# vitskvara/VBMatrixFactorization.jl

Hardware: AMD Instinct MI355X
Metric: VB iterations/sec (higher is better)
Workload: dtype bf16

## Files before the change

### vbmatrixfactorization.jl_amd/csrc/ctrl_kernels.hpp

```cpp
#pragma once
#include "common.hpp"
#include "blk_inverse.hpp"

namespace vbmf {

struct StateLayout {
    int Hp;
    __host__ __device__ long long n2() const { return (long long)Hp * Hp; }
    __host__ __device__ long long GA() const { return 0; }
    __host__ __device__ long long GB() const { return n2(); }
    __host__ __device__ long long GD() const { return 2 * n2(); }
    __host__ __device__ long long GX() const { return 3 * n2(); }
    __host__ __device__ long long SA() const { return 3 * n2() + 8; }
    __host__ __device__ long long SB() const { return 4 * n2() + 8; }
    __host__ __device__ long long KB() const { return 5 * n2() + 8; }
    __host__ __device__ long long W0() const { return 6 * n2() + 8; }
    __host__ __device__ long long W1() const { return 7 * n2() + 8; }
    __host__ __device__ long long W2() const { return 8 * n2() + 8; }
    __host__ __device__ long long ca() const { return 9 * n2() + 8; }
    __host__ __device__ long long cb() const { return 9 * n2() + 8 + Hp; }
    __host__ __device__ long long scal() const { return 9 * n2() + 8 + 2 * Hp; }
    __host__ __device__ long long total() const { return scal() + 32; }
};
enum : int { S_SIGMA2 = 0, S_TRYY, S_LOGDET_SA, S_LOGDET_SB, S_LAMB_PREV, S_LAMB_NEW, S_LAMD, S_D, S_ELBO,
// ... 429 lines not shown
        double theta = 0.0, theta_prev = 0.0, a0 = 0.0;
        bool again = false;
        for (int j = 0; j < kmax; ++j) {
            const float4* v4 = reinterpret_cast<const float4*>(&vbuf[cq * 16]);
            f32x2v a2[RB];
#pragma unroll
            for (int r = 0; r < RB; ++r) a2[r] = f32x2v{0.f, 0.f};
#pragma unroll
            for (int jj = 0; jj < 4; ++jj) {
                const float4 v = v4[jj];
                const f32x2v va = {v.x, v.y}, vb = {v.z, v.w};
#pragma unroll
                for (int r = 0; r < RB; ++r) {
                    a2[r] = __builtin_elementwise_fma(g[r][2 * jj], va, a2[r]);
                    a2[r] = __builtin_elementwise_fma(g[r][2 * jj + 1], vb, a2[r]);
                }
            }
            float acc[RB];
#pragma unroll
            for (int r = 0; r < RB; ++r) acc[r] = rowN_sum<NCQ>(a2[r][0] + a2[r][1]);
            float mine = acc[0];
            if constexpr (RB == 4) mine = (cq & 3) == 0 ? acc[0] : ((cq & 3) == 1 ? acc[1] : ((cq & 3) == 2 ? acc[2] : acc[3]));
            double wv = owner ? (double)mine : 0.0;
            const double alpha = block_sum_dpp<NT>(q * wv, red);
            wv = owner ? wv - alpha * q - beta * qp : 0.0;
            const double b2 = block_sum_dpp<NT>(wv * wv, red);
            const int k = j + 1;
            if (t == 0) { al[j] = alpha; be2[k] = b2; }
            if (j == 0) a0 = alpha;
            const bool brk = !(b2 > 1e-28) || !(b2 > EIG_LANCZOS_EXHAUSTED * a0 * a0);
            again = brk && k < kmax;
            qp = q;
            beta = sqrt(b2);
            q = brk ? 0.0 : wv / beta;
            if (owner) vbuf[myrow] = (float)q;
            __syncthreads();
            if (brk || k == next_look || k == kmax) {
                theta = tri_lambda_max(al, be2, k, theta_prev > 1e-9 ? theta_prev - 1e-9 : 0.0, 1.0 + 1e-6, imin, 4);
                if (brk || k == kmax || theta - theta_prev <= EIG_LANCZOS_TOL * theta) break;
                theta_prev = theta;
                next_look = k < 48 ? k + 12 : (k < 64 ? 64 : (k < 128 ? k + 32 : k + 64));
            }
        }
        best = theta > best ? theta : best;
        if (!again) break;
    }
    __syncthreads();
    return best;
}

constexpr int EIG_NSQ = 10;

template <int R>
__device__ __forceinline__ void eig_squaring_dev(double* __restrict__ st, StateLayout lay, int H, int spectral, int which,
                                        const int* __restrict__ ints, float* ldsf, int slot, bool check_stop = true) {
    __shared__ double red[16];
    __shared__ int s_arg;
    if (check_stop && load_stop(ints)) return;
    const int Hp = lay.Hp;
    const double* G = st + (which == 0 ? lay.GD() : lay.GB());
    double* scal = st + lay.scal();
    double tr = 0.0;
    for (int i = threadIdx.x; i < H; i += ctrl_nthreads()) tr += G[(long long)i * Hp + i];
    tr = block_sum(tr, red);
    if (!spectral || !(tr > 0.0) || !isfinite(tr)) {
        if (threadIdx.x == 0) scal[slot] = tr;
        return;
    }
    constexpr int T = 16, NP = T * R, LD = NP + 4;
    float* A0 = ldsf;
    float* A1 = ldsf + NP * LD;
    const int tx = threadIdx.x % T, ty = threadIdx.x / T;
    for (int t = threadIdx.x; t < NP * NP; t += ctrl_nthreads()) {
        const int i = t / NP, j = t - i * NP;
        A0[i * LD + j] = (i < H && j < H) ? (float)(G[(long long)i * Hp + j] / tr) : 0.f;
    }
    __syncthreads();
    float* cur = A0;
    float* nxt = A1;
    for (int sq = 0; sq < EIG_NSQ; ++sq) {
        float c[R][R];
#pragma unroll
        for (int a = 0; a < R; ++a)
#pragma unroll
            for (int b = 0; b < R; ++b) c[a][b] = 0.f;
        for (int k = 0; k < NP; k += 4) {
            float4 ai[R], bj[R];
#pragma unroll
            for (int a = 0; a < R; ++a) ai[a] = *reinterpret_cast<const float4*>(cur + (ty + T * a) * LD + k);
#pragma unroll
            for (int b = 0; b < R; ++b) bj[b] = *reinterpret_cast<const float4*>(cur + (tx + T * b) * LD + k);
#pragma unroll
            for (int a = 0; a < R; ++a)
#pragma unroll
                for (int b = 0; b < R; ++b) {
                    c[a][b] = fmaf(ai[a].x, bj[b].x, c[a][b]);
                    c[a][b] = fmaf(ai[a].y, bj[b].y, c[a][b]);
                    c[a][b] = fmaf(ai[a].z, bj[b].z, c[a][b]);
                    c[a][b] = fmaf(ai[a].w, bj[b].w, c[a][b]);
                }
        }
        double ss = 0.0;
#pragma unroll
        for (int a = 0; a < R; ++a)
#pragma unroll
            for (int b = 0; b < R; ++b) ss += (double)c[a][b] * (double)c[a][b];
        ss = block_sum(ss, red);
        const float sc = (ss > 0.0) ? (float)(1.0 / sqrt(ss)) : 0.f;
#pragma unroll
        for (int a = 0; a < R; ++a)
#pragma unroll
            for (int b = 0; b < R; ++b) nxt[(ty + T * a) * LD + tx + T * b] = c[a][b] * sc;
        __syncthreads();
        float* tmp = cur; cur = nxt; nxt = tmp;
        if (sq > 0 && fabs(ss - 1.0) < 1e-5) break;
    }
    if (threadIdx.x < 64) {
        float best = -1.f; int arg = 0;
        for (int i = threadIdx.x; i < H; i += 64) { const float v = cur[i * LD + i]; if (v > best) { best = v; arg = i; } }
        for (int off = 32; off > 0; off >>= 1) {
            const float ob = __shfl_down(best, off); const int oa = __shfl_down(arg, off);
            if (ob > best) { best = ob; arg = oa; }
        }
        if (threadIdx.x == 0) s_arg = arg;
    }
    __syncthreads();
    double num = 0.0, den = 0.0;
    {
        const int i = threadIdx.x >> 2, q = threadIdx.x & 3;
        for (int i0 = 0; i0 < H; i0 += 64) {
            const int row = i0 + i;
            if (row < H) {
                const int jn = (H + 3) / 4, j0 = q * jn, j1 = min(H, j0 + jn);
                double acc = 0.0;
                for (int j = j0; j < j1; ++j) acc += G[(long long)row * Hp + j] * (double)cur[j * LD + s_arg];
                const double vi = (double)cur[row * LD + s_arg];
                num += vi * acc;
                if (q == 0) den += vi * vi;
            }
        }
    }
    num = block_sum(num, red);
    den = block_sum(den, red);
    if (threadIdx.x == 0) scal[slot] = den > 0.0 ? num / den : 0.0;
    __syncthreads();
}

template <int R>
__device__ __forceinline__ void eig_dev(double* __restrict__ st, StateLayout lay, int H, int spectral, int which,
                                        const int* __restrict__ ints, float* ldsf, int slot, bool check_stop = true) {
    if (R <= 4 && __builtin_expect(!(spectral & 2), 1)) {
        eig_squaring_dev<R>(st, lay, H, spectral & 1, which, ints, ldsf, slot, check_stop);
    } else {
        __shared__ double red[16];
        if (check_stop && load_stop(ints)) return;
        const int Hp = lay.Hp;
        const double* G = st + (which == 0 ? lay.GD() : lay.GB());
        double* scal = st + lay.scal();
        double tr = 0.0;
        for (int i = threadIdx.x; i < H; i += ctrl_nthreads()) tr += G[(long long)i * Hp + i];
        tr = block_sum(tr, red);
        if (!(spectral & 1) || !(tr > 0.0) || !isfinite(tr)) {
            if (threadIdx.x == 0) scal[slot] = tr;
            return;
        }
        const double theta = lanczos_lambda_max<16 * R, 256>(G, Hp, H, tr, ldsf);
        if (threadIdx.x == 0) scal[slot] = tr * theta;
    }
}

template <int R>
__global__ __launch_bounds__(256) void eig_kernel(double* __restrict__ st, StateLayout lay, int H, int spectral,
                                                  int do_d, int do_b, const int* __restrict__ ints) {
    extern __shared__ __attribute__((aligned(16))) float lds_eig[];
    const int which = blockIdx.x;
    if ((which == 0 && !do_d) || (which == 1 && !do_b)) return;
    eig_dev<R>(st, lay, H, spectral, which, ints, lds_eig, which == 0 ? S_LAMD : S_LAMB_NEW);
}

__global__ __launch_bounds__(1024) void eig_lanczos_kernel(double* __restrict__ st, StateLayout lay, int H, int spectral,
                                                           int do_d, int do_b, const int* __restrict__ ints) {
    __shared__ double red[16];
    __shared__ __attribute__((aligned(16))) unsigned char lds_lz[EIG_LDS_BYTES];
    if (load_stop(ints)) return;
    const int which = blockIdx.x;
    if ((which == 0 && !do_d) || (which == 1 && !do_b)) return;
    const int Hp = lay.Hp;
    const double* G = st + (which == 0 ? lay.GD() : lay.GB());
    double* scal = st + lay.scal();
    const int slot = which == 0 ? S_LAMD : S_LAMB_NEW;
    double tr = 0.0;
    for (int i = threadIdx.x; i < H; i += (int)blockDim.x) tr += G[(long long)i * Hp + i];
    tr = block_sum(tr, red);
    if (!(spectral & 1) || !(tr > 0.0) || !isfinite(tr)) {
        if (threadIdx.x == 0) scal[slot] = tr;
        return;
    }
    const double theta = lanczos_lambda_max<256, 1024>(G, Hp, H, tr, lds_lz);
    if (threadIdx.x == 0) scal[slot] = tr * theta;
}

struct EndHandOff {
    double* img; int np;
    double sigma2, ca_h;
    bool live;
};
__device__ __forceinline__ void ctrl_end_dev(double* __restrict__ st, StateLayout lay, int H, double Lg, double M,
                                             int flags, double eps, double* __restrict__ trace,
                                             int* __restrict__ ints, int it_row, EndHandOff& ho, bool handoff,
                                             int* __restrict__ hw = nullptr) {
    __shared__ double red[16];
    __shared__ double sc_s[32];
    __shared__ double dg[4][256];
    const int Hp = lay.Hp;
    const double* GA = st + lay.GA();
    const double* GB = st + lay.GB();
    const double* SA = st + lay.SA();
    const double* SB = st + lay.SB();
    double* ca = st + lay.ca();
    double* cb = st + lay.cb();
    double* scal = st + lay.scal();
    int stopped = load_stop(ints);
    if ((flags & 64) && stopped == it_row + 1) stopped = 0;
    const int hme = threadIdx.x;
    const double scv = hme < 32 ? scal[hme] : 0.0;
    const double trdot = st[lay.GX()];
    double ca_h = hme < H ? ca[hme] : 1.0, cb_h = hme < H ? cb[hme] : 1.0;

    double t2 = 0.0;
    {
// ... 41 lines not shown
    ho.sigma2 = sigma2; ho.ca_h = ca_h;
    if (threadIdx.x == 0) {
        const double PI2 = 6.283185307179586476925286766559;
        double F = -(Lg * M / 2.0) * log(PI2 * sigma2) - resid / (2.0 * sigma2) + e;
        F += (M / 2.0) * sc_s[S_LOGDET_SA] + M * H / 2.0 + (Lg / 2.0) * sc_s[S_LOGDET_SB] + Lg * H / 2.0;
        scal[S_SIGMA2] = sigma2;
        scal[S_ELBO] = F;
        scal[S_RESID] = resid;
        scal[S_TRYBA] = trYBA;
        if (flags & 64) {
            if (trace) { trace[4 * it_row + 1] = sigma2; trace[4 * it_row + 2] = F; trace[4 * it_row + 3] = resid; }
        } else if (flags & 8) {
            const double d = sqrt(sc_s[S_LAMD] / sc_s[S_LAMB_PREV]);
            scal[S_D] = d;
            if (!(flags & 32)) scal[S_LAMB_PREV] = sc_s[S_LAMB_NEW];
            const int it = ints[I_ITERS];
            if (trace) { trace[4 * it + 0] = d; trace[4 * it + 1] = sigma2; trace[4 * it + 2] = F; trace[4 * it + 3] = resid; }
            ints[I_ITERS] = it + 1;
            const bool rerr = stop_on_remote_error(st, lay, ints);
            const bool stop = !(d > eps) || it + 1 >= ints[I_NITER] || rerr;
            if (stop) __hip_atomic_store(ints + I_STOP, 1, __ATOMIC_RELAXED, __HIP_MEMORY_SCOPE_AGENT);
            publish_loop_words(hw, ints, stop ? 1 : 0, it + 1);
        }
    }
    __syncthreads();
}

__device__ __forceinline__ void ctrl_end_dev(double* __restrict__ st, StateLayout lay, int H, double Lg, double M,
                                             int flags, double eps, double* __restrict__ trace,
                                             int* __restrict__ ints, int* __restrict__ hw) {
    EndHandOff none{nullptr, 0, 0.0, 1.0, false};
    ctrl_end_dev(st, lay, H, Lg, M, flags, eps, trace, ints, -1, none, false, hw);
}

__global__ __launch_bounds__(1024) void ctrl_end_kernel(double* __restrict__ st, StateLayout lay, int H, double Lg,
                                                       double M, int flags, double eps,
                                                       double* __restrict__ trace, int* __restrict__ ints,
                                                       int* __restrict__ hw) {
    ctrl_end_dev(st, lay, H, Lg, M, flags, eps, trace, ints, hw);
}

#ifndef VBMF_SEAM_STAMPS
#define VBMF_SEAM_STAMPS 0
#endif
template <int R>
__device__ __forceinline__ void cov_a_after_end_dev(double* __restrict__ st, StateLayout lay, int H, const EndHandOff& ho,
                                                    float* __restrict__ S32, int* __restrict__ ints) {
    constexpr int LD = 16 * R + 2;
#if VBMF_SEAM_STAMPS
    const unsigned long long s0 = wall_clock64();
#endif
    if ((int)threadIdx.x < H) ho.img[threadIdx.x * LD + threadIdx.x] += ho.sigma2 / ho.ca_h;
    double ldK; int badK;
#if VBMF_SEAM_STAMPS
    __syncthreads();
    const unsigned long long s1 = wall_clock64();
#endif
    spd_sweep_lds4<R>(ho.img, H, &ldK, &badK);
#if VBMF_SEAM_STAMPS
    __syncthreads();
    const unsigned long long s2 = wall_clock64();
#endif
    cov_store_lds4<R>(st, lay, H, 0, ho.sigma2, S32, ints, ho.img, ldK, badK, true);
#if VBMF_SEAM_STAMPS
    __syncthreads();
    if (threadIdx.x == 0) {
        unsigned long long* stamp = reinterpret_cast<unsigned long long*>(ints + 8);
        stamp[4] = s1 - s0; stamp[5] = s2 - s1; stamp[6] = wall_clock64() - s2;
    }
#endif
}

template <int R>
__device__ __forceinline__ void commit_cov_b_dev(double* __restrict__ st, StateLayout lay, int H, double M,
                                                 float* __restrict__ S32, int* __restrict__ ints, double* W) {
    if (load_stop(ints)) return;
#if VBMF_SEAM_STAMPS
    const unsigned long long s0 = wall_clock64();
#endif
    constexpr int NP = 16 * R, LD = NP + 2, U = 16;
    const int Hp = lay.Hp, sh = 31 - __clz(Hp), n = Hp * Hp;
    const double* src = st + lay.W0();
    const double* GA = st + lay.GA();
    const double* cb = st + lay.cb();
    double* dst = st + lay.SA();
    double* scal = st + lay.scal();
    const double sigma2 = scal[S_SIGMA2];
    const double cb_t = (int)threadIdx.x < H ? cb[threadIdx.x] : 1.0;
    for (int e0 = threadIdx.x; e0 < n; e0 += U * 256) {
        double sa[U], ga[U];
#pragma unroll
        for (int u = 0; u < U; ++u) {
            const int e = e0 + u * 256;
            const int ee = e < n ? e : 0;
            sa[u] = src[ee]; ga[u] = GA[ee];
        }
#pragma unroll
        for (int u = 0; u < U; ++u) {
            const int e = e0 + u * 256;
            if (e >= n) continue;
            const int i = e >> sh, j = e & (Hp - 1);
            dst[e] = sa[u];
            if (i < NP && j < NP) W[i * LD + j] = (i < H && j < H) ? ga[u] + M * sa[u] : (i == j ? 1.0 : 0.0);
        }
    }
    __syncthreads();
    if ((int)threadIdx.x < H) W[threadIdx.x * LD + threadIdx.x] += sigma2 / cb_t;
    if (threadIdx.x == 0) {
        scal[S_LOGDET_SA] = scal[S_LOGDET_SA_SHADOW];
        scal[S_LAMB_PREV] = scal[S_LAMB_SHADOW];
    }
    double ldK; int badK;
#if VBMF_SEAM_STAMPS
    __syncthreads();
    const unsigned long long s1 = wall_clock64();
#endif
    spd_sweep_lds4<R>(W, H, &ldK, &badK);
#if VBMF_SEAM_STAMPS
    __syncthreads();
    const unsigned long long s2 = wall_clock64();
#endif
    cov_store_lds4<R>(st, lay, H, 1, sigma2, S32, ints, W, ldK, badK, false);
#if VBMF_SEAM_STAMPS
    __syncthreads();
    if (threadIdx.x == 0)
        reinterpret_cast<unsigned long long*>(ints + 8)[7] = ((s1 - s0) << 40) | ((s2 - s1) << 20) | (wall_clock64() - s2);
#endif
}

struct CtrlArgs {
    double* st; StateLayout lay; int* ints; double* trace;
    float* S32;
    double Lg, M, eps;
    int H, spectral, end_flags;
    int mode;
    int it_row;
    int* sready; int sready_val;
    int* loopw;
};
enum : int { CTRL_PREV_END = 1, CTRL_COV_A = 2, CTRL_COV_B = 4, CTRL_EIG_BOLD = 8, CTRL_COMMIT_A = 16, CTRL_EIG_AHEAD = 32 };

__device__ __forceinline__ void ctrl_loop_dev(double* __restrict__ st, StateLayout lay, double eps,
                                              double* __restrict__ trace, int* __restrict__ ints, int it_row,
                                              int* __restrict__ hw) {
    if (load_stop(ints)) return;
    if (threadIdx.x == 0) {
        double* scal = st + lay.scal();
        const double d = sqrt(scal[S_LAMD] / scal[S_LAMB_PREV]);
        scal[S_D] = d;
        if (trace) trace[4 * it_row + 0] = d;
        ints[I_ITERS] = it_row + 1;
        const bool rerr = stop_on_remote_error(st, lay, ints);
        const bool stop = !(d > eps) || it_row + 1 >= ints[I_NITER] || rerr;
        if (stop) __hip_atomic_store(ints + I_STOP, it_row + 1, __ATOMIC_RELAXED, __HIP_MEMORY_SCOPE_AGENT);
        publish_loop_words(hw, ints, stop ? it_row + 1 : 0, it_row + 1);
    }
    __syncthreads();
}

template <int R, bool SEAMS = false>
__device__ __forceinline__ void ctrl_chain(const CtrlArgs& a, void* lds, int part) {
    unsigned long long* stamp = reinterpret_cast<unsigned long long*>(a.ints + 8);
    const unsigned long long t0 = wall_clock64();
    if (SEAMS && part == 2) {
        __shared__ int stop2_s;
        if (threadIdx.x == 0) {
            const int f = load_stop(a.ints);
            stop2_s = (f != 0 && f != a.it_row + 1) ? 1 : 0;
        }
        __syncthreads();
        if (stop2_s) return;
        if (a.mode & CTRL_EIG_AHEAD)
            eig_dev<R>(a.st, a.lay, a.H, a.spectral, 1, a.ints, reinterpret_cast<float*>(lds), S_LAMB_SHADOW, false);
        return;
    }
    if (part == 0) {
        EndHandOff ho{reinterpret_cast<double*>(lds), 16 * R, 0.0, 1.0, false};
        const bool end_to_a = SEAMS && (a.mode & CTRL_PREV_END) && (a.mode & CTRL_COV_A);
        const bool commit_to_b = SEAMS && (a.mode & CTRL_COMMIT_A) && (a.mode & CTRL_COV_B);
        if (a.mode & CTRL_PREV_END)
            ctrl_end_dev(a.st, a.lay, a.H, a.Lg, a.M, (a.end_flags & ~8) | 64, a.eps, a.trace, a.ints, a.it_row, ho, end_to_a);
        const unsigned long long t1 = wall_clock64();
        if (end_to_a) {
            if (ho.live) cov_a_after_end_dev<R>(a.st, a.lay, a.H, ho, a.S32, a.ints);
        } else if (a.mode & CTRL_COV_A) {
            ctrl_cov_dev<R, 16>(a.st, a.lay, a.H, 0, a.Lg, a.S32, a.ints, reinterpret_cast<double*>(lds), true);
        }
        if (commit_to_b) commit_cov_b_dev<R>(a.st, a.lay, a.H, a.M, a.S32, a.ints, reinterpret_cast<double*>(lds));
        else if (a.mode & CTRL_COV_B) ctrl_cov_dev<R, 16>(a.st, a.lay, a.H, 1, a.M, a.S32, a.ints, reinterpret_cast<double*>(lds));
        if (threadIdx.x == 0) {
            const unsigned long long t2 = wall_clock64();
            if (a.mode & CTRL_PREV_END) stamp[0] = t1 - t0;
            if (a.mode & CTRL_COV_A) stamp[1] = t2 - t1;
            if (a.mode & CTRL_COV_B) stamp[3] = t2 - t1;
        }
        if (a.sready) {
            __threadfence();
            __syncthreads();
            if (threadIdx.x == 0) __hip_atomic_store(a.sready, a.sready_val, __ATOMIC_RELEASE, __HIP_MEMORY_SCOPE_AGENT);
        }
    } else {
        if (a.mode & CTRL_PREV_END) {
            eig_dev<R>(a.st, a.lay, a.H, a.spectral, 0, a.ints, reinterpret_cast<float*>(lds), S_LAMD);
            ctrl_loop_dev(a.st, a.lay, a.eps, a.trace, a.ints, a.it_row, a.loopw);
            if (threadIdx.x == 0) stamp[2] = wall_clock64() - t0;
        }
        if (a.mode & CTRL_EIG_BOLD)
            eig_dev<R>(a.st, a.lay, a.H, a.spectral, 1, a.ints, reinterpret_cast<float*>(lds), S_LAMB_PREV);
    }
}

template <int R>
__global__ __launch_bounds__(256) void ctrl_chain_kernel(CtrlArgs a) {
    extern __shared__ __attribute__((aligned(16))) unsigned char lds_chain[];
    ctrl_chain<R, true>(a, lds_chain, blockIdx.x);
}

constexpr size_t vbls_lds_bytes(int NB) { return (size_t)4 * (16 * NB) * (16 * NB + 2) * sizeof(double); }
struct VblsBag {
    const double* S; int lds;
    double trYY, M;
    double* sigma2;
    double* ca;
    double* SA; int ldsa, nsa;
    float* SA32;
    double* T;
    double* logdet;
};
template <int NB>
__device__ __forceinline__ void vbls_loop_dev(const double* st, StateLayout lay, int H, double Lg, int niter,
                                              const VblsBag& g, double* lds_vl, int* __restrict__ err) {
    __shared__ double red[16];
    __shared__ double ca_s[16 * NB], dg_s[16 * NB];
    constexpr int NP = 16 * NB, LD = NP + 2, IMG = NP * LD;
    constexpr int NOWN = (NB * NB + 3) / 4;
    double* W = lds_vl;
    double* Sm = lds_vl + IMG;
    double* SAm = lds_vl + 2 * IMG;
    double* Tm = lds_vl + 3 * IMG;
    const int lane = threadIdx.x & 63, w = __builtin_amdgcn_readfirstlane(threadIdx.x >> 6);
    const int c16 = lane & 15, q16 = lane >> 4;
    const int Hp = lay.Hp, nbu = (H + 15) >> 4;
    const double M = g.M;
    double sigma2 = *g.sigma2;
    const double trYY = g.trYY;
    const double* Sg = g.S;
    f64x4 k0[NOWN];
#pragma unroll
    for (int o = 0; o < NOWN; ++o) {
        const int b = w + 4 * o, I = b / NB, J = b % NB;
#pragma unroll
        for (int r = 0; r < 4; ++r) {
            const int i = 16 * I + q16 + 4 * r, j = 16 * J + c16;
            k0[o][r] = (b < NB * NB && i < H && j < H) ? st[lay.GB() + (long long)i * Hp + j] + Lg * st[lay.SB() + (long long)i * Hp + j] : 0.0;
        }
    }
    for (int t = threadIdx.x; t < NP * NP; t += 256) {
        const int i = t / NP, j = t % NP;
        Sm[i * LD + j] = (i < H && j < H) ? Sg[(long long)i * g.lds + j] : 0.0;
    }
    if (threadIdx.x < NP) ca_s[threadIdx.x] = threadIdx.x < H ? g.ca[threadIdx.x] : 1.0;
    __syncthreads();
    double ldK = 0.0;
    int bad = 0;
    for (int it = 0; it < niter; ++it) {
#pragma unroll
// ... 112 lines not shown
```

### vbmatrixfactorization.jl_amd/csrc/vbmf_hip.hip

```cpp
#include "../../include/vbmf_hip.h"

#include <hip/hip_runtime.h>
#include <rccl/rccl.h>

#include <algorithm>
#include <chrono>
#include <cmath>
#include <cstdio>
#include <cstring>
#include <string>
#include <thread>
#include <type_traits>
#include <vector>

#include "common.hpp"
#include "ctx_cache.hpp"
#include "ctx_mem.hpp"
#include "ctrl_kernels.hpp"
#include "post_kernels.hpp"
#include "rng.hpp"
#include "sparse_kernels.hpp"
#include "stream_gemm.hpp"
#include "tile_kernels.hpp"
#include "prep_kernels.hpp"
// ... 251 lines not shown
        const double R_CU = NH <= 2 ? 24e9 : (NH == 4 ? 20e9 : 10e9), R_HBM = 5.4e12;
        const double total = (double)d.XT * 32.0 * (double)ks_min * kstep * ybytes;
        const double out_bytes = (double)Hp * d.XT * 32.0 * 4.0;
        const int ns_max = (int)std::max<int64_t>(1, std::min<int64_t>(64, ks_min / (2 * kq)));
        double best = 1e300;
        ns = 1;
        for (int cand = 1; cand <= ns_max; ++cand) {
            const int blocks = bps * cand;
            const int rounds = (blocks + NUM_CU - 1) / NUM_CU;
            const double slab = cand > 1 ? cand * out_bytes * (1.0 / R_HBM + 1.0 / 1.5e12) : 0.0;
            const double t = std::max(rounds * (total / blocks) / R_CU, total / R_HBM) + slab;
            if (t < best * 0.999) { best = t; ns = cand; }
        }
    }
    if (want_splits <= 0 && NH == 8 && two_rounds_at_nh8 && bps * ns <= NUM_CU && 2 * ns <= ks_min / (2 * kq)) ns *= 2;
    ns = (int)std::max<int64_t>(1, std::min<int64_t>(ns, std::max<int64_t>(1, ks_min / kq)));
    d.nsplit = ns;
    d.steps_per_split = (int)rup(cdiv(ks_min, d.nsplit), kq);
    d.KS = d.steps_per_split * d.nsplit;
}

static void prof_begin(vbmf_ctx* c, int pass) {
    c->prof_skip = true;
    if (!c->prof) return;
    if ((c->prof_seen[pass]++ % c->prof) != 0) return;
    c->prof_skip = false;
    ProfEvent e{};
    e.pass = pass;
    hipEventCreate(&e.a);
    hipEventCreate(&e.b);
    hipEventRecord(e.a, c->stream);
    c->pev.push_back(e);
}
static void prof_end(vbmf_ctx* c) {
    if (!c->prof || c->prof_skip) return;
    hipEventRecord(c->pev.back().b, c->stream);
}
static void prof_harvest(vbmf_ctx* c) {
    for (auto& e : c->pev) {
        hipEventSynchronize(e.b);
        float ms = 0.f;
        hipEventElapsedTime(&ms, e.a, e.b);
        c->prof_ms[e.pass] += ms;
        c->prof_n[e.pass] += 1;
        hipEventDestroy(e.a);
        hipEventDestroy(e.b);
    }
    c->pev.clear();
}

static int spectral_arg(const vbmf_ctx* c) {
    return ((c->o.reference_compat & VBMF_COMPAT_SPECTRAL_DELTA) ? 1 : 0) | (c->exact_lambda ? 2 : 0);
}
static bool use_lds8(const vbmf_ctx* c) { return c->lds8 && c->NH >= 4 && c->mode == MODE_BF16X2; }

static size_t ctrl_lds_bytes_r(int R) {
    const size_t NP = 16 * (size_t)R;
    const size_t eig = std::max(R <= 4 ? (size_t)2 * NP * (NP + 4) * sizeof(float) : (size_t)0, (size_t)EIG_LDS_BYTES);
    return std::max(eig, spd_inverse_lds_bytes(R));
}
static size_t ctrl_lds_bytes(int NH) { return NH <= 4 ? ctrl_lds_bytes_r(2 * NH) : 0; }
constexpr size_t full_a_wave_lds_bytes(int NBK, int NW) { return ((size_t)NW * 16 * NBK * (16 * NBK + 2) + (size_t)NW * 16 * NBK) * sizeof(double); }
static bool fused_ctrl(const vbmf_ctx* c) { return c->in_run && c->NH <= 4; }
static int* loop_words(const vbmf_ctx* c) { return c->in_run ? c->loopw_dev : nullptr; }

struct Side {
    const Dims& d;
    const float* S;
    float* Fac;
    uint4* Ft;
    const unsigned char* mask;
    int hstart;
};
enum BSlot { B_CUR = 0, B_NEXT = 1 };
static Side side_of(vbmf_ctx* c, int which, BSlot slot) {
    if (which == 0) return Side{c->d1, c->SA32, c->A32, c->FA, c->has_mask ? c->mask : nullptr, (int)(c->H - c->H1)};
    return Side{c->d2, c->SB32, c->B32[c->bcur ^ (int)slot], c->FB, nullptr, (int)(c->H - c->H1)};
}

static CtrlArgs ctrl_args(vbmf_ctx* c, int mode, float* S32) {
    CtrlArgs ca{};
    ca.st = c->st; ca.lay = c->lay; ca.ints = c->ints; ca.trace = c->run_trace;
    ca.S32 = S32;
    ca.Lg = (double)c->Lg; ca.M = (double)c->M; ca.eps = c->run_eps;
    ca.H = (int)c->H; ca.spectral = spectral_arg(c);
    ca.end_flags = c->run_flags; ca.mode = mode; ca.it_row = (int)c->ends_enqueued; ca.loopw = loop_words(c);
    return ca;
}

static int launch_stream(vbmf_ctx* c, int pass, int ctrl_mode = 0, bool epi = false, int* epi_slabs = nullptr, bool frag_out = false) {
    const Dims& d = pass == 0 ? c->d1 : c->d2;
    const uint4* Y = pass == 0 ? c->Y1 : c->Y2;
    const uint4* F = pass == 0 ? (c->diagvar ? c->FBs : c->FB) : c->FA;
    float* out = pass == 0 ? c->P : c->Q;
    const long long ld = (long long)d.XT * 32;
    int XG = d.XT / nxw_of(c->NH, c->narrow);
    int bps = (XG + 3) / 4;
    EpiArgs ea{};
    if (epi) {
        int nb = bps;
        if (c->epi_balance && cdiv(XG, 3) <= NUM_CU) nb = cdiv(XG, 3);
        else if (c->epi_balance && cdiv(XG, NUM_CU) <= 4) nb = std::max(bps, std::min(NUM_CU, XG));
        ea.g_base = XG / nb;
        ea.g_rem = XG % nb;
        bps = nb;
        XG = 4 * nb;
    }
    const int xper = (d.nsplit > 1 && c->xcd_map) ? cdiv(bps * d.nsplit, 8) : 0;
    const int grid = (xper ? 8 * xper : bps * d.nsplit) + (ctrl_mode ? 2 : 0);
    CtrlArgs ca = ctrl_args(c, ctrl_mode, pass == 0 ? c->SA32 : c->SB32);
    ea.frag_out = frag_out ? 1 : 0;
    if (epi) {
        c->sready_seq = (c->sready_seq + 1) & 0x3fffffff;
        ea.S = c->SB32; ea.Fac = c->B32[c->bcur ^ 1]; ea.Prev = c->B32[c->bcur]; ea.Ft = c->FB; ea.slabs = c->gslab;
        ea.sready = c->ints + I_SREADY; ea.expect = ctrl_mode ? c->sready_seq + c->epi_expect_skew : -1; ea.err = c->ints + I_ERR;
        ea.spin_limit = c->epi_spin_limit;
        ea.store_fac = c->in_run ? 0 : 1;
        ea.trpart = c->trpart;
        ea.stamp = reinterpret_cast<unsigned long long*>(c->ints + 16);
        c->ntr = 4 * bps;
        if (c->in_run) c->cache.B32_store_skipped();
        if (ctrl_mode) { ca.sready = c->ints + I_SREADY; ca.sready_val = c->sready_seq; }
        if (epi_slabs) *epi_slabs = bps;
        GSLAB_CHECK(c, bps, 2 * (c->NH * (c->NH + 1) / 2) * 1024);
    }
    const size_t lds = ctrl_mode ? ctrl_lds_bytes(c->NH) : 0;
    c->frag_last[pass] = frag_out && !epi;
    if (pass == 1) c->epi_last = epi;
    prof_begin(c, pass);
    bool ok = true;
    if (use_lds8(c) && !epi) {
        if (lds > (size_t)LDS8_BYTES) FAIL(c, VBMF_ERR_INVALID, "internal: control chain needs %zu bytes of LDS", lds);
        const bool sk = pass == 1 && frag_out && c->sk_per > 0 && d.nsplit == 1;
        const int sk_per = sk ? c->sk_grid : 0;
        const float* out2 = sk ? reinterpret_cast<const float*>(c->sk_list) : nullptr;
        const int grid8 = sk ? c->sk_grid + (ctrl_mode ? 2 : 0) : grid;
        const int xper8 = sk ? 0 : xper;
        ok = dispatch<4, 8>(c->NH, [&](auto nh) {
            return dispatch<0, 1>(sk ? 1 : 0, [&](auto skc) {
                constexpr int NHc = decltype(nh)::value;
                hipLaunchKernelGGL((stream_lds8_kernel<NHc, StreamCfg<NHc>::Rc, decltype(skc)::value != 0>), dim3(grid8), dim3(512), LDS8_BYTES,
                                   c->stream, Y, F, out, d.XT, d.KS, d.steps_per_split, d.nsplit, ld, c->ints + I_STOP, ca, xper8,
                                   ea.frag_out, sk_per, out2);
            });
        });
        if (sk && c->sk_ntail > 0) {
            const long long blk = (long long)(c->NH == 8 ? 8 : 16) * c->NH * 1024;
            hipLaunchKernelGGL(streamk_fixup_kernel, dim3(16, std::min(c->sk_ntail, 1024)), dim3(256), 0, c->stream, out, c->sk_per, c->sk_tail,
                               c->sk_ntail, blk, (long long)c->Hp * c->Lp, c->ints + I_STOP);
        }
    } else {
        ok = dispatch<MODE_F32, MODE_BF16, MODE_BF16X2>(c->mode, [&](auto md) {
            constexpr int MODEc = decltype(md)::value;
            if (epi) return dispatch<1, 2>(c->NH, [&](auto nh) {
                constexpr int NHc = decltype(nh)::value;
                using Cfg = StreamCfg<NHc>;
                constexpr int DYc = NHc == 1 ? Cfg::DYc : VBMF_EPI_DY;
                hipLaunchKernelGGL((stream_gemm_kernel<MODEc, NHc, Cfg::NXWc, DYc, Cfg::DFc, Cfg::Rc, 0, 1>), dim3(grid), dim3(256), lds,
                                   c->stream, Y, F, out, XG, d.KS, d.steps_per_split, d.nsplit, ld, c->ints + I_STOP, ca, xper, ea);
            });
            if (c->narrow) return dispatch<1, 2>(c->NH, [&](auto nh) {
                constexpr int NHc = decltype(nh)::value;
                using Cfg = NarrowCfg<NHc>;
                hipLaunchKernelGGL((stream_gemm_kernel<MODEc, NHc, Cfg::NXWc, Cfg::DYc, Cfg::DFc, Cfg::Rc>), dim3(grid), dim3(256), lds,
                                   c->stream, Y, F, out, XG, d.KS, d.steps_per_split, d.nsplit, ld, c->ints + I_STOP, ca, xper, ea);
            });
            return dispatch<1, 2, 4, 8>(c->NH, [&](auto nh) {
                constexpr int NHc = decltype(nh)::value;
                using Cfg = StreamCfg<NHc>;
                hipLaunchKernelGGL((stream_gemm_kernel<MODEc, NHc, Cfg::NXWc, Cfg::DYc, Cfg::DFc, Cfg::Rc>), dim3(grid), dim3(256), lds,
                                   c->stream, Y, F, out, XG, d.KS, d.steps_per_split, d.nsplit, ld, c->ints + I_STOP, ca, xper, ea);
            });
// ... 197 lines not shown
        });
    }
    if (!ok) NO_KERNEL(c);
    return gram_reduce_tail(c, which, gated, ntr, pair_slabs, nchunk);
}

static int ctrl_threads(int H) { return H <= 16 ? 64 : (H <= 32 ? 256 : 1024); }

static hipStream_t ctrl_stream(vbmf_ctx* c) { return c->use_side ? c->side : c->stream; }
static int side_fork(vbmf_ctx* c) {
    HIPCHK(c, hipEventRecord(c->ev_main, c->stream));
    HIPCHK(c, hipStreamWaitEvent(c->side, c->ev_main, 0));
    c->use_side = true;
    return VBMF_OK;
}
static int side_end(vbmf_ctx* c) {
    c->use_side = false;
    HIPCHK(c, hipEventRecord(c->ev_side, c->side));
    c->side_pending = true;
    return VBMF_OK;
}
static int side_join(vbmf_ctx* c) {
    if (!c->side_pending) return VBMF_OK;
    HIPCHK(c, hipStreamWaitEvent(c->stream, c->ev_side, 0));
    c->side_pending = false;
    return VBMF_OK;
}
static bool side_overlap(const vbmf_ctx* c) { return c->in_run && c->NH == 8; }

template <int R, int T>
constexpr size_t cov_lds_bytes() { return (R == 8 && T == 32) ? (size_t)(INV256_LDS_DOUBLES + 256) * sizeof(double) : spd_inverse_lds_bytes(R); }

static int launch_ctrl_cov(vbmf_ctx* c, int which) {
    const double N = which == 0 ? (double)c->Lg : (double)c->M;
    float* S32 = which == 0 ? c->SA32 : c->SB32;
    ctrl_tier(c->H, [&](auto r, auto t) {
        constexpr int R = decltype(r)::value, T = decltype(t)::value;
        hipLaunchKernelGGL((ctrl_cov_kernel<R, T>), dim3(1), dim3(T * T), (cov_lds_bytes<R, T>()), ctrl_stream(c), c->st, c->lay, (int)c->H, which,
                           N, S32, c->ints);
    });
    HIPCHK(c, hipGetLastError());
    return VBMF_OK;
}

static int launch_eig(vbmf_ctx* c, int do_d, int do_b) {
    const int H = (int)c->H, spectral = spectral_arg(c);
    hipStream_t s = ctrl_stream(c);
    ctrl_tier(H, [&](auto r, auto t) {
        constexpr int R = decltype(r)::value, NP = 16 * R;
        if constexpr (decltype(t)::value == 32) {
            hipLaunchKernelGGL(eig_lanczos_kernel, dim3(2), dim3(1024), 0, s, c->st, c->lay, H, spectral, do_d, do_b, c->ints);
        } else {
            const size_t lds = std::max(R <= 4 ? (size_t)2 * NP * (NP + 4) * sizeof(float) : (size_t)0, (size_t)EIG_LDS_BYTES);
            hipLaunchKernelGGL((eig_kernel<R>), dim3(2), dim3(256), lds, s, c->st, c->lay, H, spectral, do_d, do_b, c->ints);
        }
    });
    HIPCHK(c, hipGetLastError());
    return VBMF_OK;
}

static int launch_ctrl_end(vbmf_ctx* c, int flags, double eps, double* trace) {
    hipLaunchKernelGGL(ctrl_end_kernel, dim3(1), dim3(c->H > 128 ? 1024 : 256), 0, ctrl_stream(c), c->st, c->lay, (int)c->H, (double)c->Lg,
                       (double)c->M, flags, eps, trace, c->ints, loop_words(c));
    HIPCHK(c, hipGetLastError());
    return VBMF_OK;
}

static int ensure_B(vbmf_ctx* c);
static int ensure_ready(vbmf_ctx* c, bool need_Y = true, bool want_B = true) {
    if (need_Y && !c->cache.have_Y()) FAIL(c, VBMF_ERR_INVALID, "no Y: call vbmf_set_Y or vbmf_set_Y_synthetic first");
    if (!c->cache.have_state()) FAIL(c, VBMF_ERR_INVALID, "no state: call vbmf_set_state first");
    if (c->o.nranks > 1 && !c->comm_ready) FAIL(c, VBMF_ERR_COMM, "nranks > 1 but vbmf_comm_init was not called");
    if (want_B) TRY(ensure_B(c));
    if (c->cache.have_Y() && !c->cache.trYY_reduced()) {
        double* dst = c->st + c->lay.scal() + S_TRYY;
        HIPCHK(c, hipMemcpyAsync(dst, &c->trYY_local, sizeof(double), hipMemcpyHostToDevice, c->stream));
        HIPCHK(c, hipStreamSynchronize(c->stream));
        TRY(allreduce_sum(c, dst, 1, true));
        c->cache.trYY_summed();
    }
    if (c->diagvar && c->cache.have_noise() && !c->cache.noise_mean_reduced()) {
        if (sharded(c)) TRY(allreduce_sum(c, c->st + c->lay.scal() + S_SIGMA2, 1, true));
        c->cache.noise_mean_summed();
    }
    return VBMF_OK;
}

static int ensure_gram_A(vbmf_ctx* c) {
    if (c->cache.gram_A()) return VBMF_OK;
    TRY(launch_gram(c, 0, c->A32, nullptr, false));
    c->cache.gram_A_made();
    return VBMF_OK;
}
static int ensure_gram_B(vbmf_ctx* c) {
    if (c->cache.gram_B()) return VBMF_OK;
    TRY(launch_gram(c, 1, c->B32[c->bcur], nullptr, false));
    c->cache.gram_B_made();
    return VBMF_OK;
}

static int do_update_A(vbmf_ctx* c, bool reuse_P = false) {
    TRY(ensure_gram_B(c));
    const bool have_P = reuse_P && c->cache.P();
    bool commit_pending = false;
    if (have_P) {
        TRY(launch_ctrl_cov(c, 0));
    } else if (fused_ctrl(c)) {
// ... 173 lines not shown
    HIPCHK(c, le);
    HIPCHK(c, se);
    c->gram_build_ms = ms;
    c->cache.G_built();
    return VBMF_OK;
}

static int gram_product(vbmf_ctx* c, bool partials) {
    const int* stop = c->ints + I_STOP;
    const int KT = 2 * c->GT;
    const int64_t Mp1 = (int64_t)c->d1.XT * 32;
    const long long n = (long long)c->Hp * Mp1;
    const float* Wo = c->W32g[c->wcur];
    float* Wn = c->W32g[c->wcur ^ 1];
    const dim3 wg(cdiv(KT, GW_KS));
    const bool ok = dispatch<32, 64, 128, 256>(c->Hp, [&](auto hp) {
        constexpr int HPT = decltype(hp)::value, HPc = HPT == 256 ? 128 : HPT;
        if constexpr (HPT == 256)
            hipLaunchKernelGGL((gram_w_cols_kernel<256, 2>), dim3(wg.x, 2), dim3(512), 0, c->stream, c->A32, c->SB32, Wo, Wn, c->Wt, (long long)c->M, KT, stop);
        else
            hipLaunchKernelGGL((gram_w_kernel<HPT>), wg, dim3(HPT * 4), 0, c->stream, c->A32, c->SB32, Wo, Wn, c->Wt, (long long)c->M, KT, stop);
        float* out = c->g_nsplit > 1 ? c->gslabs : c->gPQ;
        const dim3 grid(c->g_nrg * c->g_nsplit, c->NH / gram_prod_nh(c));
        prof_begin(c, 0);
        {
            constexpr int NHT = HPT / 32, NHc = NHT == 8 ? 4 : NHT;
            hipLaunchKernelGGL((gram_prod_kernel<NHc, NHT>), grid, dim3(GramProd<NHc>::THREADS), GramProd<NHc>::LDS_BYTES, c->stream,
                               reinterpret_cast<const float4*>(c->Gt), c->Wt, out, c->GT, c->d1.XT, c->g_sps, c->g_nrg, n, 2 * n, stop);
        }
        prof_end(c);
        if (!partials) {
            if (c->g_nsplit > 1)
                hipLaunchKernelGGL(slab_sum_kernel, dim3(grid_for(2 * n / 4, 256, 2048)), dim3(256), 0, c->stream, c->gslabs, c->g_nsplit, 2 * n,
                                   c->gPQ, 2 * n, stop, SideCopy{});
            return;
        }
        const dim3 tg((HPT == 256 ? 8 : 2) * c->g_nchunk);
        hipLaunchKernelGGL((gram_tail_kernel<HPc, HPT>), tg, dim3(512), 0, c->stream, out, c->g_nsplit, 2 * n, c->gPQ, n, (long long)Mp1, Wn, Wo,
                           c->A32, (long long)c->M, c->g_rpc, c->g_nchunk, c->g_part, stop);
        const dim3 rg(cdiv(2 * (int64_t)c->Hp * c->Hp + 1, GRED_E));
        hipLaunchKernelGGL((gram_part_reduce_kernel<HPc, HPT>), rg, dim3(256), 0, c->stream, c->g_part, c->g_nchunk, c->st, c->lay, stop);
    });
    if (!ok) FAIL(c, VBMF_ERR_INVALID, "internal: the Gram-form sweep covers Hp <= 256");
    HIPCHK(c, hipGetLastError());
    return VBMF_OK;
}

static int launch_chain(vbmf_ctx* c, int mode, float* S32) {
    if (c->H > 128) FAIL(c, VBMF_ERR_INVALID, "internal: the stand-alone control chain covers H <= 128");
    const CtrlArgs ca = ctrl_args(c, mode, S32);
    const int parts = (mode & CTRL_EIG_AHEAD) ? 3 : ((mode & (CTRL_PREV_END | CTRL_EIG_BOLD)) ? 2 : 1);
    ctrl_tier(c->H, [&](auto r, auto t) {
        constexpr int R = decltype(r)::value;
        if constexpr (decltype(t)::value == 16)
            hipLaunchKernelGGL((ctrl_chain_kernel<R>), dim3(parts), dim3(256), ctrl_lds_bytes_r(R), c->stream, ca);
    });
    HIPCHK(c, hipGetLastError());
    return VBMF_OK;
}

static int gram_sweep(vbmf_ctx* c) {
    TRY(launch_chain(c, CTRL_COV_A | CTRL_EIG_AHEAD | (c->tail_pending ? CTRL_PREV_END : 0), c->SA32));
    if (c->tail_pending) ++c->ends_enqueued;
    c->tail_pending = false;
    c->P_frag = true;
    if (fused_gram(c)) TRY(launch_post_gram(c, 0, c->gPQ));
    else {
        TRY(launch_post_frag(c, 0, c->gPQ));
        TRY(launch_gram(c, 0, c->A32, nullptr, true));
    }
    TRY(launch_chain(c, CTRL_COMMIT_A | CTRL_COV_B, c->SB32));
    TRY(gram_product(c, true));
    c->wcur ^= 1;
    c->cache.gram_sweep_done_basic();
    return VBMF_OK;
}

static int prepare_trYBA(vbmf_ctx* c, int* flag) {
    *flag = 0;
    if (c->cache.tr()) return VBMF_OK;
    double* dst = c->st + c->lay.GX();
    HIPCHK(c, hipMemsetAsync(dst, 0, sizeof(double), c->stream));
    if (c->cache.P()) {
        const float* In = (sharded(c) || c->d1.nsplit > 1) ? c->Pred : c->P;
        const int ns = 1;
        const long long ld = (long long)c->d1.XT * 32;
        const int g = grid_for(c->M, 256, 1024);
        hipLaunchKernelGGL(dot_kernel, dim3(g), dim3(256), 0, c->stream, In, ld, ns,
                           (long long)c->Hp * ld, c->A32, c->Hp, (long long)c->M, c->ypart, c->P_frag ? c->NH : 0);
        hipLaunchKernelGGL(sum_partials_kernel, dim3(1), dim3(256), 0, c->stream, c->ypart, g, dst);
    } else {
        TRY(launch_stream(c, 1));
        const long long ld = (long long)c->d2.XT * 32;
        const int g = grid_for(c->L, 256, 1024);
        hipLaunchKernelGGL(dot_kernel, dim3(g), dim3(256), 0, c->stream, c->Q, ld, c->d2.nsplit,
                           (long long)c->Hp * ld, c->B32[c->bcur], c->Hp, (long long)c->L, c->ypart, 0);
        hipLaunchKernelGGL(sum_partials_kernel, dim3(1), dim3(256), 0, c->stream, c->ypart, g, dst);
        if (sharded(c)) TRY(allreduce_sum(c, dst, 1, true));
    }
    HIPCHK(c, hipGetLastError());
    c->cache.tr_made();
    return VBMF_OK;
}

static double d_resolution(const vbmf_ctx* c) { return c->mode == MODE_F32 ? 2e-6 : (c->mode == MODE_BF16X2 ? 1e-5 : 4e-3); }
static void run_note_eps(vbmf_ctx* c, int64_t niter, double eps, int64_t done, double d) {
    c->err.clear();
    if (done >= niter && eps > 0.0 && d > eps && eps < d_resolution(c)) {
// ... 2264 lines not shown
```

Before: 4758.

## Exploit symmetry in eig matrix squaring with 512-thread upper-triangle tiling

The repeated-squaring eigenvalue estimate now computes only the upper-triangular blocks of the symmetric 64x64 product. The work is spread over 10 half-wave tiles in a 512-thread block, with software-pipelined float4 LDS loads and inline v_fmac. The 256 owner threads then rebuild the full matrix by mirroring before normalisation. The eig and control-chain kernels are launched with 512 threads for R==4, which raises launch bounds and may affect register pressure in other parts of the chain. The chain part-0 path drops its extra threads.

```diff
diff --git a/vbmatrixfactorization.jl_amd/csrc/ctrl_kernels.hpp b/vbmatrixfactorization.jl_amd/csrc/ctrl_kernels.hpp
--- a/vbmatrixfactorization.jl_amd/csrc/ctrl_kernels.hpp
+++ b/vbmatrixfactorization.jl_amd/csrc/ctrl_kernels.hpp
@@ -505,8 +505,59 @@
 constexpr int EIG_NSQ = 10;
 
 template <int R>
+__device__ __forceinline__ void eig_square_tri(const float* __restrict__ cur, float* __restrict__ nxt) {
+    static_assert(R == 4, "thread tiles of 2 x 4 on a 64 x 64 matrix");
+    constexpr int TR = R / 2, TC = R, NP = 16 * R, LD = NP + 4;
+    const int hw = threadIdx.x >> 5;
+    if (hw >= 10) return;
+    const int Ib = hw < 4 ? 0 : (hw < 7 ? 1 : (hw < 9 ? 2 : 3));
+    const int Jb = hw < 4 ? hw : (hw < 7 ? hw - 3 : (hw < 9 ? hw - 5 : 3));
+    const int l = threadIdx.x & 31;
+    const int i0 = (8 * Ib + (l >> 2)) * TR, j0 = (4 * Jb + (l & 3)) * TC;
+    float c[TR][TC];
+#pragma unroll
+    for (int a = 0; a < TR; ++a)
+#pragma unroll
+        for (int b = 0; b < TC; ++b) c[a][b] = 0.f;
+    const float* pa = cur + i0 * LD;
+    const float* pb = cur + j0 * LD;
+    float4 ai[2][TR], bj[2][TC];
+    auto load = [&](int s, int k) {
+#pragma unroll
+        for (int a = 0; a < TR; ++a) ai[s][a] = *reinterpret_cast<const float4*>(pa + a * LD + k);
+#pragma unroll
+        for (int b = 0; b < TC; ++b) bj[s][b] = *reinterpret_cast<const float4*>(pb + b * LD + k);
+        __builtin_amdgcn_sched_barrier(0);
+    };
+    auto mac = [&](int s) {
+#pragma unroll
+        for (int a = 0; a < TR; ++a)
+#pragma unroll
+            for (int b = 0; b < TC; ++b) {
+                asm("v_fmac_f32 %0, %1, %2" : "+v"(c[a][b]) : "v"(ai[s][a].x), "v"(bj[s][b].x));
+                asm("v_fmac_f32 %0, %1, %2" : "+v"(c[a][b]) : "v"(ai[s][a].y), "v"(bj[s][b].y));
+                asm("v_fmac_f32 %0, %1, %2" : "+v"(c[a][b]) : "v"(ai[s][a].z), "v"(bj[s][b].z));
+                asm("v_fmac_f32 %0, %1, %2" : "+v"(c[a][b]) : "v"(ai[s][a].w), "v"(bj[s][b].w));
+            }
+        __builtin_amdgcn_sched_barrier(0);
+    };
+    load(0, 0);
+#pragma unroll
+    for (int k = 0; k < NP; k += 8) {
+        load(1, k + 4);
+        mac(0);
+        if (k + 8 < NP) load(0, k + 8);
+        mac(1);
+    }
+#pragma unroll
+    for (int a = 0; a < TR; ++a)
+#pragma unroll
+        for (int b = 0; b < TC; ++b) nxt[(i0 + a) * LD + j0 + b] = c[a][b];
+}
+
+template <int R>
 __device__ __forceinline__ void eig_squaring_dev(double* __restrict__ st, StateLayout lay, int H, int spectral, int which,
-                                        const int* __restrict__ ints, float* ldsf, int slot, bool check_stop = true) {
+                                        const int* __restrict__ ints, float* ldsf, int slot, bool check_stop, bool wide) {
     __shared__ double red[16];
     __shared__ int s_arg;
     if (check_stop && load_stop(ints)) return;
@@ -524,7 +575,7 @@
     float* A0 = ldsf;
     float* A1 = ldsf + NP * LD;
     const int tx = threadIdx.x % T, ty = threadIdx.x / T;
-    for (int t = threadIdx.x; t < NP * NP; t += ctrl_nthreads()) {
+    for (int t = threadIdx.x; t < NP * NP; t += wide ? 512 : ctrl_nthreads()) {
         const int i = t / NP, j = t - i * NP;
         A0[i * LD + j] = (i < H && j < H) ? (float)(G[(long long)i * Hp + j] / tr) : 0.f;
     }
@@ -533,37 +584,56 @@
     float* nxt = A1;
     for (int sq = 0; sq < EIG_NSQ; ++sq) {
         float c[R][R];
-#pragma unroll
-        for (int a = 0; a < R; ++a)
-#pragma unroll
-            for (int b = 0; b < R; ++b) c[a][b] = 0.f;
-        for (int k = 0; k < NP; k += 4) {
-            float4 ai[R], bj[R];
-#pragma unroll
-            for (int a = 0; a < R; ++a) ai[a] = *reinterpret_cast<const float4*>(cur + (ty + T * a) * LD + k);
-#pragma unroll
-            for (int b = 0; b < R; ++b) bj[b] = *reinterpret_cast<const float4*>(cur + (tx + T * b) * LD + k);
+        if (wide) {
+            if constexpr (R == 4) eig_square_tri<R>(cur, nxt);
+            __syncthreads();
+            if (threadIdx.x < 256) {
+#pragma unroll
+                for (int a = 0; a < R; ++a)
+#pragma unroll
+                    for (int b = 0; b < R; ++b) {
+                        const int i = ty + T * a, j = tx + T * b;
+                        c[a][b] = nxt[min(i, j) * LD + max(i, j)];
+                    }
+            }
+        } else {
 #pragma unroll
             for (int a = 0; a < R; ++a)
 #pragma unroll
-                for (int b = 0; b < R; ++b) {
-                    c[a][b] = fmaf(ai[a].x, bj[b].x, c[a][b]);
-                    c[a][b] = fmaf(ai[a].y, bj[b].y, c[a][b]);
-                    c[a][b] = fmaf(ai[a].z, bj[b].z, c[a][b]);
-                    c[a][b] = fmaf(ai[a].w, bj[b].w, c[a][b]);
-                }
-        }
+                for (int b = 0; b < R; ++b) c[a][b] = 0.f;
+            for (int k = 0; k < NP; k += 4) {
+                float4 ai[R], bj[R];
+#pragma unroll
+                for (int a = 0; a < R; ++a) ai[a] = *reinterpret_cast<const float4*>(cur + (ty + T * a) * LD + k);
+#pragma unroll
+                for (int b = 0; b < R; ++b) bj[b] = *reinterpret_cast<const float4*>(cur + (tx + T * b) * LD + k);
+#pragma unroll
+                for (int a = 0; a < R; ++a)
+#pragma unroll
+                    for (int b = 0; b < R; ++b) {
+                        c[a][b] = fmaf(ai[a].x, bj[b].x, c[a][b]);
+                        c[a][b] = fmaf(ai[a].y, bj[b].y, c[a][b]);
+                        c[a][b] = fmaf(ai[a].z, bj[b].z, c[a][b]);
+                        c[a][b] = fmaf(ai[a].w, bj[b].w, c[a][b]);
+                    }
+            }
+        }
+        const bool owner = !wide || threadIdx.x < 256;
         double ss = 0.0;
-#pragma unroll
-        for (int a = 0; a < R; ++a)
-#pragma unroll
-            for (int b = 0; b < R; ++b) ss += (double)c[a][b] * (double)c[a][b];
+        if (owner) {
+#pragma unroll
+            for (int a = 0; a < R; ++a)
+#pragma unroll
+                for (int b = 0; b < R; ++b) ss += (double)c[a][b] * (double)c[a][b];
+        }
         ss = block_sum(ss, red);
         const float sc = (ss > 0.0) ? (float)(1.0 / sqrt(ss)) : 0.f;
-#pragma unroll
-        for (int a = 0; a < R; ++a)
-#pragma unroll
-            for (int b = 0; b < R; ++b) nxt[(ty + T * a) * LD + tx + T * b] = c[a][b] * sc;
+        if (owner) {
+#pragma unroll
+            for (int a = 0; a < R; ++a)
+#pragma unroll
+                for (int b = 0; b < R; ++b) nxt[(ty + T * a) * LD + tx + T * b] = c[a][b] * sc;
+        }
         __syncthreads();
         float* tmp = cur; cur = nxt; nxt = tmp;
         if (sq > 0 && fabs(ss - 1.0) < 1e-5) break;
@@ -599,11 +669,12 @@
     __syncthreads();
 }
 
-template <int R>
+template <int R, bool WIDE_OK = false>
 __device__ __forceinline__ void eig_dev(double* __restrict__ st, StateLayout lay, int H, int spectral, int which,
                                         const int* __restrict__ ints, float* ldsf, int slot, bool check_stop = true) {
     if (R <= 4 && __builtin_expect(!(spectral & 2), 1)) {
-        eig_squaring_dev<R>(st, lay, H, spectral & 1, which, ints, ldsf, slot, check_stop);
+        const bool wide = WIDE_OK && R == 4 && blockDim.x == 512u;
+        eig_squaring_dev<R>(st, lay, H, spectral & 1, which, ints, ldsf, slot, check_stop, wide);
     } else {
         __shared__ double red[16];
         if (check_stop && load_stop(ints)) return;
@@ -623,12 +694,12 @@
 }
 
 template <int R>
-__global__ __launch_bounds__(256) void eig_kernel(double* __restrict__ st, StateLayout lay, int H, int spectral,
+__global__ __launch_bounds__(R == 4 ? 512 : 256) void eig_kernel(double* __restrict__ st, StateLayout lay, int H, int spectral,
                                                   int do_d, int do_b, const int* __restrict__ ints) {
     extern __shared__ __attribute__((aligned(16))) float lds_eig[];
     const int which = blockIdx.x;
     if ((which == 0 && !do_d) || (which == 1 && !do_b)) return;
-    eig_dev<R>(st, lay, H, spectral, which, ints, lds_eig, which == 0 ? S_LAMD : S_LAMB_NEW);
+    eig_dev<R, true>(st, lay, H, spectral, which, ints, lds_eig, which == 0 ? S_LAMD : S_LAMB_NEW);
 }
 
 __global__ __launch_bounds__(1024) void eig_lanczos_kernel(double* __restrict__ st, StateLayout lay, int H, int spectral,
@@ -776,10 +847,6 @@
 #endif
     if ((int)threadIdx.x < H) ho.img[threadIdx.x * LD + threadIdx.x] += ho.sigma2 / ho.ca_h;
     double ldK; int badK;
-#if VBMF_SEAM_STAMPS
-    __syncthreads();
-    const unsigned long long s1 = wall_clock64();
-#endif
     spd_sweep_lds4<R>(ho.img, H, &ldK, &badK);
 #if VBMF_SEAM_STAMPS
     __syncthreads();
@@ -790,7 +857,7 @@
     __syncthreads();
     if (threadIdx.x == 0) {
         unsigned long long* stamp = reinterpret_cast<unsigned long long*>(ints + 8);
-        stamp[4] = s1 - s0; stamp[5] = s2 - s1; stamp[6] = wall_clock64() - s2;
+        stamp[5] = s2 - s0; stamp[6] = wall_clock64() - s2;
     }
 #endif
 }
@@ -895,10 +962,14 @@
         __syncthreads();
         if (stop2_s) return;
         if (a.mode & CTRL_EIG_AHEAD)
-            eig_dev<R>(a.st, a.lay, a.H, a.spectral, 1, a.ints, reinterpret_cast<float*>(lds), S_LAMB_SHADOW, false);
+            eig_dev<R, SEAMS>(a.st, a.lay, a.H, a.spectral, 1, a.ints, reinterpret_cast<float*>(lds), S_LAMB_SHADOW, false);
+#if VBMF_SEAM_STAMPS
+        if (threadIdx.x == 0) stamp[4] = wall_clock64() - t0;
+#endif
         return;
     }
     if (part == 0) {
+        if (SEAMS && threadIdx.x >= 256) return;
         EndHandOff ho{reinterpret_cast<double*>(lds), 16 * R, 0.0, 1.0, false};
         const bool end_to_a = SEAMS && (a.mode & CTRL_PREV_END) && (a.mode & CTRL_COV_A);
         const bool commit_to_b = SEAMS && (a.mode & CTRL_COMMIT_A) && (a.mode & CTRL_COV_B);
@@ -925,17 +996,17 @@
         }
     } else {
         if (a.mode & CTRL_PREV_END) {
-            eig_dev<R>(a.st, a.lay, a.H, a.spectral, 0, a.ints, reinterpret_cast<float*>(lds), S_LAMD);
+            eig_dev<R, SEAMS>(a.st, a.lay, a.H, a.spectral, 0, a.ints, reinterpret_cast<float*>(lds), S_LAMD);
             ctrl_loop_dev(a.st, a.lay, a.eps, a.trace, a.ints, a.it_row, a.loopw);
             if (threadIdx.x == 0) stamp[2] = wall_clock64() - t0;
         }
         if (a.mode & CTRL_EIG_BOLD)
-            eig_dev<R>(a.st, a.lay, a.H, a.spectral, 1, a.ints, reinterpret_cast<float*>(lds), S_LAMB_PREV);
+            eig_dev<R, SEAMS>(a.st, a.lay, a.H, a.spectral, 1, a.ints, reinterpret_cast<float*>(lds), S_LAMB_PREV);
     }
 }
 
 template <int R>
-__global__ __launch_bounds__(256) void ctrl_chain_kernel(CtrlArgs a) {
+__global__ __launch_bounds__(R == 4 ? 512 : 256) void ctrl_chain_kernel(CtrlArgs a) {
     extern __shared__ __attribute__((aligned(16))) unsigned char lds_chain[];
     ctrl_chain<R, true>(a, lds_chain, blockIdx.x);
 }
diff --git a/vbmatrixfactorization.jl_amd/csrc/vbmf_hip.hip b/vbmatrixfactorization.jl_amd/csrc/vbmf_hip.hip
--- a/vbmatrixfactorization.jl_amd/csrc/vbmf_hip.hip
+++ b/vbmatrixfactorization.jl_amd/csrc/vbmf_hip.hip
@@ -327,6 +327,7 @@
 static int spectral_arg(const vbmf_ctx* c) {
     return ((c->o.reference_compat & VBMF_COMPAT_SPECTRAL_DELTA) ? 1 : 0) | (c->exact_lambda ? 2 : 0);
 }
+static int eig_wide_launch(int R, int spectral) { return (R == 4 && !(spectral & 2)) ? 512 : 256; }
 static bool use_lds8(const vbmf_ctx* c) { return c->lds8 && c->NH >= 4 && c->mode == MODE_BF16X2; }
 
 static size_t ctrl_lds_bytes_r(int R) {
@@ -392,7 +393,11 @@
         ea.spin_limit = c->epi_spin_limit;
         ea.store_fac = c->in_run ? 0 : 1;
         ea.trpart = c->trpart;
+#if VBMF_SEAM_STAMPS
+        ea.stamp = nullptr;
+#else
         ea.stamp = reinterpret_cast<unsigned long long*>(c->ints + 16);
+#endif
         c->ntr = 4 * bps;
         if (c->in_run) c->cache.B32_store_skipped();
         if (ctrl_mode) { ca.sready = c->ints + I_SREADY; ca.sready_val = c->sready_seq; }
@@ -696,7 +701,8 @@
             hipLaunchKernelGGL(eig_lanczos_kernel, dim3(2), dim3(1024), 0, s, c->st, c->lay, H, spectral, do_d, do_b, c->ints);
         } else {
             const size_t lds = std::max(R <= 4 ? (size_t)2 * NP * (NP + 4) * sizeof(float) : (size_t)0, (size_t)EIG_LDS_BYTES);
-            hipLaunchKernelGGL((eig_kernel<R>), dim3(2), dim3(256), lds, s, c->st, c->lay, H, spectral, do_d, do_b, c->ints);
+            hipLaunchKernelGGL((eig_kernel<R>), dim3(2), dim3(eig_wide_launch(R, spectral)), lds, s, c->st, c->lay, H, spectral, do_d, do_b,
+                               c->ints);
         }
     });
     HIPCHK(c, hipGetLastError());
@@ -976,8 +982,9 @@
     const int parts = (mode & CTRL_EIG_AHEAD) ? 3 : ((mode & (CTRL_PREV_END | CTRL_EIG_BOLD)) ? 2 : 1);
     ctrl_tier(c->H, [&](auto r, auto t) {
         constexpr int R = decltype(r)::value;
+        const int nthr = (mode & (CTRL_PREV_END | CTRL_EIG_AHEAD | CTRL_EIG_BOLD)) ? eig_wide_launch(R, ca.spectral) : 256;
         if constexpr (decltype(t)::value == 16)
-            hipLaunchKernelGGL((ctrl_chain_kernel<R>), dim3(parts), dim3(256), ctrl_lds_bytes_r(R), c->stream, ca);
+            hipLaunchKernelGGL((ctrl_chain_kernel<R>), dim3(parts), dim3(nthr), ctrl_lds_bytes_r(R), c->stream, ca);
     });
     HIPCHK(c, hipGetLastError());
     return VBMF_OK;
```

After: 4828 (median of 6 runs). +1.5%, better.
